# hideki1217/rusTfhe

Hardware: AMD Instinct MI355X
Metric: HomNAND gates/sec (whole node), N=1024 (higher is better)
Workload: dtype f64

## Files before the change

rustfhe_amd/csrc/rtfhe_body_pair.hpp:

```cpp
    constexpr int LOGN = 10;
    typedef Geo<LOGN> G;
    constexpr int N = G::N, P = G::P, R = G::R, NT = 128 * GATES;
    constexpr uint32_t M = decomp_mask(L, BGBIT);
    static_assert(L == 3, "three rows per side are held in registers");
    extern __shared__ __align__(16) unsigned char smem[];
    const int tid = threadIdx.x, lane = tid & 63;
    const int wave = __builtin_amdgcn_readfirstlane(tid >> 6);
    const int slot = wave % GATES;
    const int side = wave / GATES;
    cplx* tw = reinterpret_cast<cplx*>(smem);
    for (int idx = tid; idx < G::TW_TOTAL; idx += NT) tw[idx] = a.tw[idx];
    const cplx* twf = tw;
    const cplx* twi = tw + G::TW_DIR;

    const int g_raw = blockIdx.x * GATES + slot;
    const int g = g_raw < a.count ? g_raw : a.count - 1;
    const GateIo io = gate_io(a, g);
    const auto tv = tv_row(tvs, g, N);
    const bool live = g_raw < a.count && io.ok && tv.ok();

    unsigned char* gbase = smem + PairLds::TW + (size_t)slot * PairLds::gate_bytes(a.npad);
    uint32_t* accbuf = reinterpret_cast<uint32_t*>(gbase);
    uint32_t* abar = accbuf + 2 * N;
    double* xb0 = reinterpret_cast<double*>(gbase + (size_t)2 * N * 4 + (size_t)a.npad * 4);
    uint32_t* flags = reinterpret_cast<uint32_t*>(gbase + PairLds::gate_bytes(a.npad) - PairLds::FLAGS);
    if (lane == 0) flags[side] = 0u;
    const unsigned my_flag = (unsigned)__builtin_amdgcn_readfirstlane((int)(unsigned)(size_t)(__attribute__((address_space(3))) uint32_t*)(flags + side));
    const unsigned partner_flag = (unsigned)__builtin_amdgcn_readfirstlane((int)(unsigned)(size_t)(__attribute__((address_space(3))) uint32_t*)(flags + (1 - side)));
    double* xb1 = xb0 + 2 * G::XSLOTS;
    double* myx = side ? xb1 : xb0;
    cplx* hand0 = reinterpret_cast<cplx*>(xb0) + lane;
    cplx* hand1 = reinterpret_cast<cplx*>(xb1) + lane;
    uint32_t* poly = accbuf + side * N;

    const int n = a.n;
    {
        constexpr int SH = 32 - LOGN - 1;
        for (int i = lane + 64 * side; i <= n; i += 128) {
            const uint32_t t = gate_linear(io.op, io.p0[i], io.p1[i], i == n);
            if constexpr (decltype(tvs)::MANY) abar[i] = mod_switch<SH>(t, i == n, tv_shift(tvs));
            else abar[i] = (i == n) ? (t >> SH) : ((t + (1u << (SH - 1))) >> SH);
        }
    }
    __syncthreads();
    {
        const int bbar = (int)abar[n];
#pragma unroll
        for (int mm = 0; mm < 2 * R; mm++) {
            const int c = lane + 64 * mm;
            const int e = (c + bbar) & (2 * N - 1);
            if constexpr (decltype(tvs)::ENC) poly[c] = side ? tv_word_a<LOGN>(tv, e) : tv_word<LOGN>(tv, e);
            else poly[c] = side ? 0u : tv_word<LOGN>(tv, e);
        }
    }
    wave_lds_sync();
    uint32_t own[2 * R];
#pragma unroll
    for (int mm = 0; mm < 2 * R; mm++) own[mm] = poly[lane + 64 * mm];

#ifdef RTFHE_WG_STAMPS
    unsigned long long tsum[16] = {0, 0, 0, 0, 0, 0, 0, 0, 0, 0, 0, 0, 0, 0, 0, 0}, tprev = __builtin_amdgcn_s_memtime();
#define PAIR_STAMP(k) do { __builtin_amdgcn_sched_barrier(0); unsigned long long t_ = __builtin_amdgcn_s_memtime(); \
        asm volatile("s_waitcnt lgkmcnt(0)" ::: "memory"); tsum[k] += t_ - tprev; tprev = t_; __builtin_amdgcn_sched_barrier(0); } while (0)
#else
#define PAIR_STAMP(k) do { } while (0)
#endif
    const size_t trgsw_cplx = (size_t)2 * L * 2 * R * 64;
    cplx bA[R], bB[R];
    typedef unsigned int v4u __attribute__((ext_vector_type(4)));
    const __amdgpu_buffer_rsrc_t bk_rsrc = __builtin_amdgcn_make_buffer_rsrc(const_cast<cplx*>(a.bk), 0, 0x7fffffff, 0x00020000);
    const int lane16 = lane * 16;
    auto fetch = [&](cplx (&dst)[R], int step, int rc) {
        const size_t row = (size_t)step * trgsw_cplx + (size_t)((side * L + rc % L) * 2 + rc / L) * R * 64;
        const int s_lo = __builtin_amdgcn_readfirstlane((int)(row * sizeof(cplx)));
        const int s_hi = s_lo + (R / 2) * 64 * (int)sizeof(cplx);
        __builtin_amdgcn_sched_barrier(0);
#pragma unroll
        for (int m = 0; m < R / 2; m++) {
            const v4u v = __builtin_amdgcn_raw_buffer_load_b128(bk_rsrc, lane16 + m * 1024, s_lo, 0);
            dst[m] = make_double2(__longlong_as_double(((unsigned long long)v.y << 32) | v.x), __longlong_as_double(((unsigned long long)v.w << 32) | v.z));
        }
#pragma unroll
        for (int m = 0; m < R / 2; m++) {
            const v4u v = __builtin_amdgcn_raw_buffer_load_b128(bk_rsrc, lane16 + m * 1024, s_hi, 0);
            dst[R / 2 + m] = make_double2(__longlong_as_double(((unsigned long long)v.y << 32) | v.x), __longlong_as_double(((unsigned long long)v.w << 32) | v.z));
        }
        __builtin_amdgcn_sched_barrier(0);
    };
    if (a.steps > 0) {
        fetch(bA, 0, side ? 0 : 1);
        fetch(bB, 0, side ? 1 : 0);
    }
    constexpr int LOWER_AT = 2, RAISE_AT = 10;
    auto prio_point = [&](int point) {
        if (point == LOWER_AT) asm volatile("s_cmp_lg_u32 %0, 0\n\ts_cbranch_scc1 1f\n\ts_setprio 0\n1:" ::"s"(side) : "scc");
        if (point == RAISE_AT) asm volatile("s_cmp_lg_u32 %0, 0\n\ts_cbranch_scc1 1f\n\ts_setprio 2\n1:" ::"s"(side) : "scc");
    };
    if (side) __builtin_amdgcn_s_setprio(1); else __builtin_amdgcn_s_setprio(2);
#pragma unroll 1
    for (int i = 0; i < a.steps; i++) {
        const int r = __builtin_amdgcn_readfirstlane((int)abar[i]);
        const int nxt = (i + 1 < a.steps) ? i + 1 : i;
        int ln = lane;
        asm volatile("" : "+v"(ln));
        uint32_t u[2 * R];
#pragma unroll
        for (int mm = 0; mm < 2 * R; mm++) {
            const int c = ln + 64 * mm;
            u[mm] = ((rotated_coef<LOGN>(poly, c, r) - own[mm]) + M) ^ M;
        }
        PAIR_STAMP(0);
        double xr[L][R], xi[L][R];
#pragma unroll
        for (int jj = 0; jj < L; jj++) {
#pragma unroll
            for (int m = 0; m < R; m++) {
                xr[jj][m] = (double)decomp_digit(u[m], BGBIT, jj);
                xi[jj][m] = (double)decomp_digit(u[R + m], BGBIT, jj);
            }
        }
        auto pp1 = [&]() { prio_point(1); };
        fft_forward_multi_a<LOGN, L, true, decltype(pp1), true>(xr, xi, twf, myx, myx + G::XSLOTS, ln, pp1);
        prio_point(2);
        PAIR_STAMP(1);
        fft_forward_multi_b<LOGN, L, BOOT_TRIV>(xr, xi, twf);
        prio_point(5);
        PAIR_STAMP(3);

        double sre[R], sim[R];
        auto zero = [&]() {
#pragma unroll
            for (int m = 0; m < R; m++) { sre[m] = 0.0; sim[m] = 0.0; }
        };
        auto put = [&](cplx* h) {
#pragma unroll
            for (int m = 0; m < R; m++) h[m * 64] = make_double2(sre[m], sim[m]);
        };
        auto get = [&](const cplx* h) {
#pragma unroll
            for (int m = 0; m < R; m++) { const cplx v = h[m * 64]; sre[m] = v.x; sim[m] = v.y; }
        };

        if (side == 0) {
            mac_row_first<R>(sre, sim, bB, xr[0], xi[0]); fetch(bB, i, 2);
            mac_row<R>(sre, sim, bA, xr[1], xi[1]); fetch(bA, i, 3);
            mac_row<R>(sre, sim, bB, xr[2], xi[2]); fetch(bB, i, 4);
            put(hand0);
        }
        prio_point(6);
        PAIR_STAMP(4);
        flag_arrive(my_flag, 2u * (unsigned)i + 1u); flag_wait(partner_flag, 2u * (unsigned)i + 1u);
        prio_point(7);
        PAIR_STAMP(5);
        if (side == 0) zero(); else get(hand0);
        mac_row<R>(sre, sim, bA, xr[0], xi[0]); fetch(bA, i, side ? 2 : 5);
        mac_row<R>(sre, sim, bB, xr[1], xi[1]); fetch(bB, side ? i : nxt, side ? 3 : 0);
        mac_row<R>(sre, sim, bA, xr[2], xi[2]); fetch(bA, side ? i : nxt, side ? 4 : 1);
        put(side ? hand0 : hand1);
        prio_point(8);
        PAIR_STAMP(6);
        flag_arrive(my_flag, 2u * (unsigned)i + 2u); flag_wait(partner_flag, 2u * (unsigned)i + 2u);
        prio_point(9);
        PAIR_STAMP(7);
        if (side == 1) {
            get(hand1);
            mac_row<R>(sre, sim, bB, xr[0], xi[0]); fetch(bB, i, 5);
            mac_row<R>(sre, sim, bA, xr[1], xi[1]); fetch(bA, nxt, 0);
            mac_row<R>(sre, sim, bB, xr[2], xi[2]); fetch(bB, nxt, 1);
        } else {
            get(hand0);
        }
        PAIR_STAMP(8);

        fft_inverse<LOGN, 1, BOOT_TRIV>(sre, sim, twi, twi, myx, lane);
#pragma unroll
        for (int m = 0; m < R; m++) {
            const int c = lane + 64 * m;
            own[m] += trunc_to_torus(sre[m]);
            own[R + m] += trunc_to_torus(sim[m]);
            poly[c] = own[m];
            poly[c + P] = own[R + m];
        }
        wave_lds_sync();
        prio_point(10);
        PAIR_STAMP(9);
    }
    __builtin_amdgcn_s_setprio(0);
#ifdef RTFHE_WG_STAMPS
    if (a.dbg && blockIdx.x == 0 && lane == 0)
        for (int k = 0; k < 16; k++) a.dbg[wave * 16 + k] = tsum[k];
#endif

    if (a.mode == MODE_BLIND_ROTATE) {
        if (live) {
            uint32_t* o = a.out + (size_t)g * 2 * N + side * N;
            for (int c = lane; c < N; c += 64) o[c] = poly[c];
        }
        return;
    }

    if (side == 1) {
        uint32_t av[2 * R];
#pragma unroll
        for (int mm = 0; mm < 2 * R; mm++) av[mm] = poly[lane + 64 * mm];
        wave_lds_sync();
#pragma unroll
        for (int mm = 0; mm < 2 * R; mm++) {
            const int c = lane + 64 * mm;
            poly[(N - c) & (N - 1)] = (c == 0) ? av[mm] : (0u - av[mm]);
        }
    }
    __syncthreads();
    if (a.mode == MODE_EXTRACT) {
        if constexpr (decltype(tvs)::MANY) {
            if (live) many_extract<N>(a.ext, a.ext_first + g, tv_shift(tvs), accbuf, side * (N / 2) + lane, (side + 1) * (N / 2), 64, side ? -1 : lane);
            return;
        }
        if (live) {
            const int ge = a.ext_first + g;
            for (int c = side * (N / 2) + lane; c < (side + 1) * (N / 2); c += 64) *ext_slot(a.ext, ge, c, N) = accbuf[N + c];
            if (side == 0 && lane == 0) *ext_slot(a.ext, ge, N, N) = accbuf[0];
            for (int c = side * 64 + lane; c <= n; c += 128) io.out[c] = 0u;
        }
        return;
    }
    uint4 sum[KSQ];
    ks_accumulate<LOGN, KS_T, KS_BB, KSQ>(accbuf + N, side * (N / 2), (side + 1) * (N / 2), a.ksk, a.ksw, sum, lane);
    uint4* part = reinterpret_cast<uint4*>(xb1) + lane;
    if (side == 1) {
#pragma unroll
        for (int q = 0; q < KSQ; q++) part[q * 64] = sum[q];
    }
    __syncthreads();
    if (side == 0 && live) {
        const uint32_t bprime = accbuf[0];
        uint32_t* out = io.out;
#pragma unroll
        for (int q = 0; q < KSQ; q++) {
            const uint4 o = part[q * 64];
            const int col = 4 * (lane + 64 * q);
            const uint32_t s[4] = {sum[q].x + o.x, sum[q].y + o.y, sum[q].z + o.z, sum[q].w + o.w};
#pragma unroll
            for (int e = 0; e < 4; e++)
                if (col + e <= n) out[col + e] = ((col + e == n) ? bprime : 0u) - s[e];
        }
    }
```

rustfhe_amd/csrc/rtfhe_device.hpp:

```cpp
#pragma once

#include <hip/hip_runtime.h>
#include <stdint.h>

namespace rtfhe {

typedef double2 cplx;

constexpr bool BOOT_TRIV = true;

__host__ __device__ constexpr int ilog2(int v) { return v <= 1 ? 0 : 1 + ilog2(v >> 1); }

template <int LOGN>
struct Geo {
    static constexpr int N = 1 << LOGN;
    static constexpr int P = N / 2;
    static constexpr int LOGP = LOGN - 1;
    static constexpr int R = P / 64;
    static constexpr int LR = ilog2(R);
    static constexpr int LOW = LOGP - 2 * LR;
    static constexpr int NLOW = 1 << LOW;
    static_assert(LOW >= 2 && LOW <= LR, "supported: N = 1024, 2048");
    static constexpr int TW_TWIST = 0;
    static constexpr int TW_P1 = TW_TWIST + R * 64;
    static constexpr int TW_P2 = TW_P1 + (R - 1) * 64;
    static constexpr int TW_P3 = TW_P2 + (R - 1) * NLOW;
    static constexpr int TW_DIR = TW_P3 + (NLOW - 4);
    static constexpr int TW_TOTAL = 2 * TW_DIR;
    static constexpr int XSLOTS = P + 64;
    __host__ __device__ static constexpr int f1(int pos) { return pos + NLOW * (pos >> 6); }
    __host__ __device__ static constexpr int f2(int pos) { return pos + (pos >> LR); }
    __host__ __device__ static constexpr int pos1(int lane, int m) { return lane + 64 * m; }
    __host__ __device__ static constexpr int pos2(int lane, int m) {
        return ((lane >> LOW) << 6) | (m << LOW) | (lane & (NLOW - 1));
    }
    __host__ __device__ static constexpr int pos3(int lane, int m) { return (lane << LR) | m; }
};

__device__ __forceinline__ void wave_lds_sync() {
    __builtin_amdgcn_fence(__ATOMIC_RELEASE, "wavefront");
    __builtin_amdgcn_wave_barrier();
    __builtin_amdgcn_fence(__ATOMIC_ACQUIRE, "wavefront");
}

__device__ __forceinline__ void lds_st(double* p, double v) {
    __hip_atomic_store(p, v, __ATOMIC_RELAXED, __HIP_MEMORY_SCOPE_WAVEFRONT);
}
__device__ __forceinline__ double lds_ld(const double* p) {
    return __hip_atomic_load(p, __ATOMIC_RELAXED, __HIP_MEMORY_SCOPE_WAVEFRONT);
}
__device__ __forceinline__ void lds_st128(cplx* p, double re, double im) { *p = make_double2(re, im); }
__device__ __forceinline__ cplx lds_ld128(const cplx* p) { return *p; }


template <int CNT>
struct Tw {
    cplx w[CNT > 0 ? CNT : 1];
    __device__ __forceinline__ void load(const cplx* __restrict__ tw, int stride) {
#pragma unroll
        for (int e = 0; e < CNT; e++) w[e] = tw[e * stride];
    }
};

template <int R, int MB, bool TRIV0 = false>
__device__ __forceinline__ void fwd_stage_tw(double (&re)[R], double (&im)[R], const cplx* w) {
    constexpr int h = 1 << MB;
#pragma unroll
    for (int m = 0; m < R; m++) {
        if (m & h) continue;
        const int m1 = m | h, q = m & (h - 1);
        const double sr = re[m] + re[m1], si = im[m] + im[m1];
        const double dr = re[m] - re[m1], di = im[m] - im[m1];
        re[m] = sr; im[m] = si;
        if (TRIV0 && q == 0) { re[m1] = dr; im[m1] = di; continue; }
        double a = dr * w[q].x, b = di * w[q].y;
        re[m1] = a - b;
        a = dr * w[q].y; b = di * w[q].x;
        im[m1] = a + b;
    }
}

template <int R, int MB, bool CONJ = false, bool TRIV0 = false>
__device__ __forceinline__ void inv_stage_tw(double (&re)[R], double (&im)[R], const cplx* w) {
    constexpr int h = 1 << MB;
#pragma unroll
    for (int m = 0; m < R; m++) {
        if (m & h) continue;
        const int m1 = m | h, q = m & (h - 1);
        if (TRIV0 && q == 0) {
            const double ar = re[m], ai = im[m], tr = re[m1], ti = im[m1];
            re[m] = ar + tr; im[m] = ai + ti;
            re[m1] = ar - tr; im[m1] = ai - ti;
            continue;
        }
        const double t0 = re[m1] * w[q].x, t1 = re[m1] * w[q].y, t2 = im[m1] * w[q].x, t3 = im[m1] * w[q].y;
        const double tr = CONJ ? t0 + t3 : t0 - t3, ti = CONJ ? t2 - t1 : t1 + t2;
        const double ar = re[m], ai = im[m];
        re[m] = ar + tr; im[m] = ai + ti;
        re[m1] = ar - tr; im[m1] = ai - ti;
    }
}

template <int R>
__device__ __forceinline__ void stage_size2(double (&re)[R], double (&im)[R]) {
#pragma unroll
    for (int m = 0; m < R; m += 2) {
        const double r0 = re[m], r1 = re[m + 1], j0 = im[m], j1 = im[m + 1];
        re[m] = r0 + r1; re[m + 1] = r0 + (-r1);
        im[m] = j0 + j1; im[m + 1] = j0 + (-j1);
    }
}

template <int R>
__device__ __forceinline__ void fwd_stage_size4(double (&re)[R], double (&im)[R]) {
#pragma unroll
    for (int m = 0; m < R; m += 4) {
        const double r0 = re[m], r1 = re[m + 1], r2 = re[m + 2], r3 = re[m + 3];
        const double j0 = im[m], j1 = im[m + 1], j2 = im[m + 2], j3 = im[m + 3];
        re[m] = r0 + r2; re[m + 1] = r1 + r3; re[m + 2] = r0 + (-r2); re[m + 3] = (-j1) + j3;
        im[m] = j0 + j2; im[m + 1] = j1 + j3; im[m + 2] = j0 + (-j2); im[m + 3] = r1 + (-r3);
    }
}

template <int R>
__device__ __forceinline__ void inv_stage_size4(double (&re)[R], double (&im)[R]) {
#pragma unroll
    for (int m = 0; m < R; m += 4) {
        const double r0 = re[m], r1 = re[m + 1], r2 = re[m + 2], r3 = re[m + 3];
        const double j0 = im[m], j1 = im[m + 1], j2 = im[m + 2], j3 = im[m + 3];
        re[m] = r0 + r2; re[m + 1] = r1 + j3;    re[m + 2] = r0 + (-r2); re[m + 3] = r1 + (-j3);
        im[m] = j0 + j2; im[m + 1] = j1 + (-r3); im[m + 2] = j0 + (-j2); im[m + 3] = j1 + r3;
    }
}

template <int R>
__device__ __forceinline__ void twist_mul(double (&re)[R], double (&im)[R], const cplx* w) {
#pragma unroll
    for (int m = 0; m < R; m++) {
        const double rc = re[m] * w[m].x, ic = im[m] * w[m].x, rs = re[m] * w[m].y, is = im[m] * w[m].y;
        re[m] = rc - is;
        im[m] = ic + rs;
    }
}

// ... 112 lines not shown
        wave_lds_sync();
    }
}

template <int LOGN, int DUAL = 0>
__device__ __forceinline__ void fft_forward_a(double (&re)[Geo<LOGN>::R], double (&im)[Geo<LOGN>::R],
                                              const cplx* __restrict__ tw, double* __restrict__ xbuf, int lane,
                                              double* __restrict__ xim = nullptr) {
    typedef Geo<LOGN> G;
    constexpr int R = G::R;
    Tw<R> wt; Tw<R - 1> w1, w2;
    wt.load(tw + G::TW_TWIST + lane, 64);
    w1.load(tw + G::TW_P1 + lane, 64);
    twist_mul<R>(re, im, wt.w);
    P12<R, G::LR - 1>::fwd(re, im, w1.w);
    w2.load(tw + G::TW_P2 + (lane & (G::NLOW - 1)), G::NLOW);
    exchange<LOGN, 1, 2, DUAL>(re, im, xbuf, lane, xim);
    P12<R, G::LR - 1>::fwd(re, im, w2.w);
}
template <int LOGN, int DUAL = 0, bool TRIV = false>
__device__ __forceinline__ void fft_forward_b(double (&re)[Geo<LOGN>::R], double (&im)[Geo<LOGN>::R],
                                              const cplx* __restrict__ tw, double* __restrict__ xbuf, int lane,
                                              double* __restrict__ xim = nullptr) {
    typedef Geo<LOGN> G;
    Tw<G::NLOW - 4> w3;
    w3.load(tw + G::TW_P3, 1);
    exchange<LOGN, 2, 3, DUAL>(re, im, xbuf, lane, xim);
    P3<G::R, G::NLOW, G::LOW - 1, TRIV>::fwd(re, im, w3.w);
}
template <int LOGN, int DUAL = 0, bool TRIV = false>
__device__ __forceinline__ void fft_forward(double (&re)[Geo<LOGN>::R], double (&im)[Geo<LOGN>::R],
                                            const cplx* __restrict__ tw, double* __restrict__ xbuf, int lane,
                                            double* __restrict__ xim = nullptr) {
    fft_forward_a<LOGN, DUAL>(re, im, tw, xbuf, lane, xim);
    fft_forward_b<LOGN, DUAL, TRIV>(re, im, tw, xbuf, lane, xim);
}

template <int LOGN, int FROM, int TO, bool B128 = false>
struct XAffine {
    typedef Geo<LOGN> G;
    static_assert(G::LR == G::LOW, "N = 1024 geometry");
    static constexpr int R = G::R;
    static constexpr bool X12 = (FROM + TO == 3);
    __device__ __forceinline__ static int base(int layout, int lane) {
        return layout == 1 ? lane : layout == 2 ? (G::NLOW + 64) * (lane >> G::LOW) + (lane & (G::NLOW - 1)) : (R + 1) * lane;
    }
    __host__ __device__ static constexpr int stride(int layout) { return layout == 1 ? 64 + G::NLOW : layout == 2 ? (X12 ? G::NLOW : G::NLOW + 1) : 1; }
    __device__ __forceinline__ static void write(const double (&re)[R], const double (&im)[R], double* __restrict__ xbuf, double* __restrict__ xim, int lane) {
        const int bw = base(FROM, lane);
        constexpr int sw = stride(FROM);
        if constexpr (B128) {
            cplx* xc = reinterpret_cast<cplx*>(xbuf);
#pragma unroll
            for (int m = 0; m < R; m++) lds_st128(&xc[bw + sw * m], re[m], im[m]);
            return;
        }
#pragma unroll
        for (int m = 0; m < R; m++) lds_st(&xbuf[bw + sw * m], re[m]);
#pragma unroll
        for (int m = 0; m < R; m++) lds_st(&xim[bw + sw * m], im[m]);
    }
    template <int HALF>
    __device__ __forceinline__ static void read_half(double (&re)[R], double (&im)[R], const double* __restrict__ xbuf, const double* __restrict__ xim, int lane) {
        const int br = base(TO, lane);
        constexpr int sr = stride(TO);
        if constexpr (B128) {
            const cplx* xc = reinterpret_cast<const cplx*>(xbuf);
#pragma unroll
            for (int m = HALF * (R / 4); m < (HALF + 1) * (R / 4); m++) {
                const cplx a = lds_ld128(&xc[br + sr * m]), b = lds_ld128(&xc[br + sr * (m + R / 2)]);
                re[m] = a.x; im[m] = a.y; re[m + R / 2] = b.x; im[m + R / 2] = b.y;
            }
            return;
        }
#pragma unroll
        for (int m = HALF * (R / 4); m < (HALF + 1) * (R / 4); m++) {
            re[m] = lds_ld(&xbuf[br + sr * m]); re[m + R / 2] = lds_ld(&xbuf[br + sr * (m + R / 2)]);
            im[m] = lds_ld(&xim[br + sr * m]);  im[m + R / 2] = lds_ld(&xim[br + sr * (m + R / 2)]);
        }
    }
};

struct NoHook { __device__ __forceinline__ void operator()() const {} };
template <int LOGN, int NR, bool TWIST = true, typename HOOK = NoHook, bool INTERLEAVE = false, bool B128 = false>
__device__ __forceinline__ void fft_forward_multi_a(double (&re)[NR][Geo<LOGN>::R], double (&im)[NR][Geo<LOGN>::R],
                                                    const cplx* __restrict__ tw, double* __restrict__ xbuf, double* __restrict__ xim, int lane,
                                                    HOOK after_pass1 = HOOK()) {
    typedef Geo<LOGN> G;
    constexpr int R = G::R;
#pragma unroll
    for (int half = 0; half < (TWIST ? 2 : 0); half++) {
        cplx wt[R / 2];
#pragma unroll
        for (int m = 0; m < R / 2; m++) wt[m] = tw[G::TW_TWIST + lane + 64 * (half * (R / 2) + m)];
#pragma unroll
        for (int j = 0; j < NR; j++)
#pragma unroll
            for (int m = 0; m < R / 2; m++) {
                const int k = half * (R / 2) + m;
                const double rc = re[j][k] * wt[m].x, ic = im[j][k] * wt[m].x, rs = re[j][k] * wt[m].y, is = im[j][k] * wt[m].y;
                re[j][k] = rc - is;
                im[j][k] = ic + rs;
            }
    }
  if constexpr (INTERLEAVE) {
    static_assert(G::LR == 3, "three stages per pass");
    typedef XAffine<LOGN, 1, 2, B128> X1;
    typedef XAffine<LOGN, 2, 3, B128> X2;
    auto pass = [&](int j, const cplx* w, auto&& between0, auto&& between1) {
        fwd_stage_tw<R, 2>(re[j], im[j], w + (R - 8));
        __builtin_amdgcn_sched_barrier(0); between0(); __builtin_amdgcn_sched_barrier(0);
        fwd_stage_tw<R, 1>(re[j], im[j], w + (R - 4));
        __builtin_amdgcn_sched_barrier(0); between1(); __builtin_amdgcn_sched_barrier(0);
        fwd_stage_tw<R, 0>(re[j], im[j], w + (R - 2));
        __builtin_amdgcn_sched_barrier(0);
    };
    auto nothing = [] {};
    Tw<R - 1> w1;
    w1.load(tw + G::TW_P1 + lane, 64);
#pragma unroll
    for (int j = 0; j < NR; j++) {
        if (j == 0) pass(0, w1.w, nothing, nothing);
        else pass(j, w1.w, [&] { X1::template read_half<0>(re[j - 1], im[j - 1], xbuf, xim, lane); }, [&] { X1::template read_half<1>(re[j - 1], im[j - 1], xbuf, xim, lane); wave_lds_sync(); });
        X1::write(re[j], im[j], xbuf, xim, lane);
        wave_lds_sync();
    }
    after_pass1();
    Tw<R - 1> w2;
    w2.load(tw + G::TW_P2 + (lane & (G::NLOW - 1)), G::NLOW);
#pragma unroll
    for (int j = 0; j < NR; j++) {
        if (j == 0) pass(0, w2.w, [&] { X1::template read_half<0>(re[NR - 1], im[NR - 1], xbuf, xim, lane); }, [&] { X1::template read_half<1>(re[NR - 1], im[NR - 1], xbuf, xim, lane); wave_lds_sync(); });
        else pass(j, w2.w, [&] { X2::template read_half<0>(re[j - 1], im[j - 1], xbuf, xim, lane); }, [&] { X2::template read_half<1>(re[j - 1], im[j - 1], xbuf, xim, lane); wave_lds_sync(); });
        X2::write(re[j], im[j], xbuf, xim, lane);
        wave_lds_sync();
    }
    X2::template read_half<0>(re[NR - 1], im[NR - 1], xbuf, xim, lane);
    X2::template read_half<1>(re[NR - 1], im[NR - 1], xbuf, xim, lane);
    wave_lds_sync();
  } else {
    {
        Tw<R - 1> w1;
        w1.load(tw + G::TW_P1 + lane, 64);
#pragma unroll
        for (int j = 0; j < NR; j++) {
            P12<R, G::LR - 1>::fwd(re[j], im[j], w1.w);
            exchange<LOGN, 1, 2, B128 ? 2 : 1>(re[j], im[j], xbuf, lane, xim);
        }
    }
    after_pass1();
    Tw<R - 1> w2;
    w2.load(tw + G::TW_P2 + (lane & (G::NLOW - 1)), G::NLOW);
#pragma unroll
    for (int j = 0; j < NR; j++) {
        P12<R, G::LR - 1>::fwd(re[j], im[j], w2.w);
        exchange<LOGN, 2, 3, B128 ? 2 : 1>(re[j], im[j], xbuf, lane, xim);
    }
  }
}
template <int LOGN, int NR, bool TRIV = false>
__device__ __forceinline__ void fft_forward_multi_b(double (&re)[NR][Geo<LOGN>::R], double (&im)[NR][Geo<LOGN>::R],
                                                    const cplx* __restrict__ tw) {
    typedef Geo<LOGN> G;
    Tw<G::NLOW - 4> w3;
    w3.load(tw + G::TW_P3, 1);
#pragma unroll
    for (int j = 0; j < NR; j++) P3<G::R, G::NLOW, G::LOW - 1, TRIV>::fwd(re[j], im[j], w3.w);
}

template <int LOGN, int DUAL = 0, bool TRIV = false>
__device__ __forceinline__ void fft_inverse(double (&re)[Geo<LOGN>::R], double (&im)[Geo<LOGN>::R],
                                            const cplx* __restrict__ tw_small, const cplx* __restrict__ tw_big,
                                            double* __restrict__ xbuf, int lane, double* __restrict__ xim = nullptr) {
    typedef Geo<LOGN> G;
    constexpr int R = G::R;
    Tw<G::NLOW - 4> w3; Tw<R - 1> w2, w1; Tw<R> wt;
    w3.load(tw_small + G::TW_P3, 1);
    P3<R, G::NLOW, G::LOW - 1, TRIV>::template inv<false>(re, im, w3.w);
    w2.load(tw_small + G::TW_P2 + (lane & (G::NLOW - 1)), G::NLOW);
    exchange<LOGN, 3, 2, DUAL>(re, im, xbuf, lane, xim);
    P12<R, G::LR - 1>::inv(re, im, w2.w);
    w1.load(tw_big + G::TW_P1 + lane, 64);
    exchange<LOGN, 2, 1, DUAL>(re, im, xbuf, lane, xim);
    wt.load(tw_big + G::TW_TWIST + lane, 64);
    P12<R, G::LR - 1>::inv(re, im, w1.w);
    twist_mul<R>(re, im, wt.w);
}

template <int LOGN>
struct TwStage {
    typedef Geo<LOGN> G;
    static constexpr bool SPLIT = (LOGN >= 11);
    static constexpr int LDS_CPLX = SPLIT ? G::TW_DIR + (G::TW_DIR - G::TW_P2) : G::TW_TOTAL;
    __device__ __forceinline__ static void stage(cplx* __restrict__ lds, const cplx* __restrict__ global, int tid, int nthreads) {
        if constexpr (SPLIT) {
            for (int idx = tid; idx < G::TW_DIR; idx += nthreads) lds[idx] = global[idx];
            for (int idx = tid + G::TW_P2; idx < G::TW_DIR; idx += nthreads) lds[G::TW_DIR + idx - G::TW_P2] = global[G::TW_DIR + idx];
        } else {
            for (int idx = tid; idx < G::TW_TOTAL; idx += nthreads) lds[idx] = global[idx];
        }
    }
    __device__ __forceinline__ static const cplx* fwd(const cplx* lds) { return lds; }
    __device__ __forceinline__ static const cplx* inv_small(const cplx* lds) { return SPLIT ? lds + G::TW_DIR - G::TW_P2 : lds + G::TW_DIR; }
    __device__ __forceinline__ static const cplx* inv_big(const cplx* lds, const cplx* global) { return SPLIT ? global + G::TW_DIR : lds + G::TW_DIR; }
};

__device__ __forceinline__ uint32_t trunc_to_torus(double x) {
    const double t = __builtin_trunc(x);
    const double y = t + 6755399441055744.0;
    return (uint32_t)__double_as_longlong(y);
}

__device__ __forceinline__ uint32_t trunc_to_torus_wide(double x) {
    const double t = __builtin_trunc(x);
    if (!(__builtin_fabs(t) < 9223372036854775808.0)) return 0u;
    const double hi = __builtin_floor(t * 2.3283064365386963e-10);
    const double lo = __builtin_fma(hi, -4294967296.0, t);
    return (uint32_t)lo;
}

__host__ __device__ constexpr uint32_t decomp_mask(int l, int bits) {
    uint32_t u = 0;
    if (32 - l * bits != 0) {
        u += 1u << (32 - l * bits - 1);
        for (int i = l; i >= 1; i--) u += 1u << (32 - i * bits - 1);
    } else {
        for (int i = l - 1; i >= 1; i--) u += 1u << (32 - i * bits - 1);
    }
    return u;
}

__device__ __forceinline__ int32_t decomp_digit(uint32_t u, int bits, int j) {
    return __builtin_amdgcn_sbfe((int32_t)u, (uint32_t)(32 - bits * (j + 1)), (uint32_t)bits);
}


__device__ __forceinline__ void flag_arrive(unsigned flag, unsigned k) {
    unsigned t0, t1;
    asm volatile("v_mov_b32 %0, %2\n\tv_mov_b32 %1, %3\n\tds_write_b32 %0, %1" : "=&v"(t0), "=&v"(t1) : "s"(flag), "s"(k) : "memory");
}
__device__ __forceinline__ void flag_wait(unsigned flag, unsigned k) {
    unsigned v, t;
    asm volatile(
        "v_mov_b32 %0, %2\n"
        "1:\n\t"
        "ds_read_b32 %0, %0\n\t"
        "s_waitcnt lgkmcnt(0)\n\t"
        "v_readfirstlane_b32 %1, %0\n\t"
        "s_sub_i32 %1, %1, %3\n\t"
        "s_cmp_lt_i32 %1, 0\n\t"
        "s_cbranch_scc0 2f\n\t"
        "s_sleep 1\n\t"
        "v_mov_b32 %0, %2\n\t"
        "s_branch 1b\n"
        "2:"
        : "=&v"(v), "=&s"(t)
        : "s"(flag), "s"(k)
        : "memory", "scc");
}
template <int LOGN>
__device__ __forceinline__ uint32_t rotated_coef(const uint32_t* __restrict__ p, int c, int r) {
    constexpr int N = 1 << LOGN;
    const int e = (c - r) & (2 * N - 1);
    const uint32_t v = p[e & (N - 1)];
    return (e >> LOGN) ? (0u - v) : v;
}

}
```

rustfhe_amd/csrc/rtfhe_kernels_pair.hpp:

```cpp
#pragma once

#include "rtfhe_kernels.hpp"


namespace rtfhe {

__device__ __forceinline__ void lds_barrier() {
    asm volatile("s_waitcnt lgkmcnt(0)\n\ts_barrier" ::: "memory");
}

__device__ __forceinline__ void pair_sync(unsigned my_flag_addr, unsigned partner_flag_addr, unsigned k) {
    asm volatile("ds_write_b32 %0, %1" ::"v"(my_flag_addr), "v"(k) : "memory");
    unsigned v;
    do {
        asm volatile("ds_read_b32 %0, %1\n\ts_waitcnt lgkmcnt(0)" : "=v"(v) : "v"(partner_flag_addr) : "memory");
        v = (unsigned)__builtin_amdgcn_readfirstlane((int)v);
    } while ((int)(v - k) < 0);
}

__device__ __forceinline__ void pair_arrive(unsigned my_flag_addr, unsigned k) {
    asm volatile("ds_write_b32 %0, %1" ::"v"(my_flag_addr), "v"(k) : "memory");
}
__device__ __forceinline__ void pair_wait(unsigned partner_flag_addr, unsigned k) {
    unsigned v;
    do {
        asm volatile("ds_read_b32 %0, %1\n\ts_waitcnt lgkmcnt(0)" : "=v"(v) : "v"(partner_flag_addr) : "memory");
        v = (unsigned)__builtin_amdgcn_readfirstlane((int)v);
    } while ((int)(v - k) < 0);
}

__device__ __forceinline__ void pair_wait_opaque(unsigned partner_flag_addr, unsigned k) {
    unsigned v, t;
    asm volatile(
        "1:\n\t"
        "ds_read_b32 %0, %2\n\t"
        "s_waitcnt lgkmcnt(0)\n\t"
        "v_readfirstlane_b32 %1, %0\n\t"
        "s_sub_i32 %1, %1, %3\n\t"
        "s_cmp_lt_i32 %1, 0\n\t"
        "s_cbranch_scc1 1b"
        : "=&v"(v), "=&s"(t)
        : "v"(partner_flag_addr), "s"(k)
        : "memory", "scc");
}

__device__ __forceinline__ void pair_wait_opaque_prio3(unsigned partner_flag_addr, unsigned k) {
    unsigned v, t;
    asm volatile(
        "1:\n\t"
        "ds_read_b32 %0, %2\n\t"
        "s_waitcnt lgkmcnt(0)\n\t"
        "v_readfirstlane_b32 %1, %0\n\t"
        "s_sub_i32 %1, %1, %3\n\t"
        "s_cmp_lt_i32 %1, 0\n\t"
        "s_cbranch_scc1 1b\n\t"
        "s_setprio 3"
        : "=&v"(v), "=&s"(t)
        : "v"(partner_flag_addr), "s"(k)
        : "memory", "scc");
}

template <int R>
__device__ __forceinline__ void mac_row_first(double (&sre)[R], double (&sim)[R], const cplx (&b)[R], const double (&re)[R], const double (&im)[R]) {
#pragma unroll
    for (int m = 0; m < R; m++) {
        const double ii = b[m].y * im[m], rr = b[m].x * re[m], ri = b[m].x * im[m], ir = b[m].y * re[m];
        sre[m] = rr - ii;
        sim[m] = ir + ri;
    }
}

template <int R>
__device__ __forceinline__ void mac_row(double (&sre)[R], double (&sim)[R], const cplx (&b)[R], const double (&re)[R], const double (&im)[R]) {
#pragma unroll
    for (int m = 0; m < R; m++) {
        const double ii = b[m].y * im[m], rr = b[m].x * re[m], ri = b[m].x * im[m], ir = b[m].y * re[m];
        sre[m] = sre[m] + (rr - ii);
        sim[m] = sim[m] + (ir + ri);
    }
}

struct PairLds {
    typedef Geo<10> G;
    static constexpr size_t TW = (size_t)G::TW_TOTAL * sizeof(cplx);
    static constexpr size_t XB = (size_t)2 * G::XSLOTS * sizeof(double);
    static_assert(XB >= (size_t)G::P * sizeof(cplx), "an exchange buffer pair must hold one spectrum");
    static constexpr size_t FLAGS = 16;
    __host__ __device__ static constexpr size_t gate_bytes(int npad) { return (size_t)2 * G::N * 4 + (size_t)npad * 4 + 2 * XB + FLAGS; }
    __host__ __device__ static constexpr size_t bytes(int gates, int npad) { return TW + (size_t)gates * gate_bytes(npad); }
};

template <int L, int BGBIT, int KS_T, int KS_BB, int KSQ, int GATES>
__global__ __launch_bounds__(128 * GATES, 1) void k_bootstrap_pair(const BootstrapArgs a) {
    const TvGate tvs{};
#include "rtfhe_body_pair.hpp"
}
template <int L, int BGBIT, int KS_T, int KS_BB, int KSQ, int GATES>
__global__ __launch_bounds__(128 * GATES, 1) void k_pbs_pair(const LutArgs<BootstrapArgs> p) {
    const BootstrapArgs& a = p.base;
    const TvLut tvs = tv_lut(p, a.fault);
#include "rtfhe_body_pair.hpp"
}
template <int L, int BGBIT, int KS_T, int KS_BB, int KSQ, int GATES>
__global__ __launch_bounds__(128 * GATES, 1) void k_pbs_many_pair(const ManyArgs<BootstrapArgs> p) {
    const BootstrapArgs& a = p.base;
    const TvMany tvs = tv_many(p, a.fault);
#include "rtfhe_body_pair.hpp"
}
template <int L, int BGBIT, int KS_T, int KS_BB, int KSQ, int GATES>
__global__ __launch_bounds__(128 * GATES, 1) void k_pbs_enc_pair(const ManyArgs<BootstrapArgs> p) {
    const BootstrapArgs& a = p.base;
    const TvEnc tvs = tv_enc(p, a.fault);
#include "rtfhe_body_pair.hpp"
}

}
```

rustfhe_amd/csrc/rtfhe_kernels_pair_rr.hpp:

```cpp
#pragma once

#include "rtfhe_kernels_pair.hpp"

namespace rtfhe {

struct PairRrLds {
    typedef Geo<10> G;
    static constexpr int SLOTS = 4, GMAX = 6;
    static constexpr size_t TW = PairLds::TW, XB = PairLds::XB;
    static constexpr size_t SLOT = 2 * XB + 16;
    static constexpr size_t DONE = 64;
    __host__ __device__ static constexpr size_t gate_bytes(int npad) { return (size_t)2 * G::N * 4 + ((size_t)npad * 2 + 15) / 16 * 16; }
    __host__ __device__ static constexpr size_t bytes(int gates, int npad) { return TW + SLOTS * SLOT + DONE + (size_t)gates * gate_bytes(npad); }
};

template <int L, int BGBIT, int KS_T, int KS_BB, int KSQ>
__global__ __launch_bounds__(512, 1) void k_bootstrap_pair_rr(const BootstrapArgs a) {
    const TvGate tvs{};
#include "rtfhe_body_pair_rr.hpp"
}
template <int L, int BGBIT, int KS_T, int KS_BB, int KSQ>
__global__ __launch_bounds__(512, 1) void k_pbs_pair_rr(const LutArgs<BootstrapArgs> p) {
    const BootstrapArgs& a = p.base;
    const TvLut tvs = tv_lut(p, a.fault);
#include "rtfhe_body_pair_rr.hpp"
}
template <int L, int BGBIT, int KS_T, int KS_BB, int KSQ>
__global__ __launch_bounds__(512, 1) void k_pbs_many_pair_rr(const ManyArgs<BootstrapArgs> p) {
    const BootstrapArgs& a = p.base;
    const TvMany tvs = tv_many(p, a.fault);
#include "rtfhe_body_pair_rr.hpp"
}
template <int L, int BGBIT, int KS_T, int KS_BB, int KSQ>
__global__ __launch_bounds__(512, 1) void k_pbs_enc_pair_rr(const ManyArgs<BootstrapArgs> p) {
    const BootstrapArgs& a = p.base;
    const TvEnc tvs = tv_enc(p, a.fault);
#include "rtfhe_body_pair_rr.hpp"
}

}
```

Baseline: 155,800.

## Keep only small FFT twiddle tables in LDS, stream large ones from global

The pair bootstrap kernel now copies only the pass-2/pass-3 twiddle tables (forward and inverse) into LDS. The large twist and pass-1 tables are read per lane directly from global memory through buffer loads. This shrinks the LDS footprint per workgroup, which may allow more gates per block or better occupancy. The cost is extra global/L2 traffic and latency on every FFT, and the rr kernel keeps the full table size.

```diff
diff --git a/rustfhe_amd/csrc/rtfhe_body_pair.hpp b/rustfhe_amd/csrc/rtfhe_body_pair.hpp
--- a/rustfhe_amd/csrc/rtfhe_body_pair.hpp
+++ b/rustfhe_amd/csrc/rtfhe_body_pair.hpp
@@ -9,9 +9,10 @@
     const int slot = wave % GATES;
     const int side = wave / GATES;
     cplx* tw = reinterpret_cast<cplx*>(smem);
-    for (int idx = tid; idx < G::TW_TOTAL; idx += NT) tw[idx] = a.tw[idx];
-    const cplx* twf = tw;
-    const cplx* twi = tw + G::TW_DIR;
+    for (int idx = tid; idx < 2 * PairLds::TW_SMALL; idx += NT)
+        tw[idx] = a.tw[idx < PairLds::TW_SMALL ? G::TW_P2 + idx : G::TW_DIR + G::TW_P2 + idx - PairLds::TW_SMALL];
+    const cplx* twf_small = tw;
+    const cplx* twi_small = tw + PairLds::TW_SMALL;
 
     const int g_raw = blockIdx.x * GATES + slot;
     const int g = g_raw < a.count ? g_raw : a.count - 1;
@@ -70,6 +71,8 @@
     typedef unsigned int v4u __attribute__((ext_vector_type(4)));
     const __amdgpu_buffer_rsrc_t bk_rsrc = __builtin_amdgcn_make_buffer_rsrc(const_cast<cplx*>(a.bk), 0, 0x7fffffff, 0x00020000);
     const int lane16 = lane * 16;
+    const __amdgpu_buffer_rsrc_t tw_rsrc = __builtin_amdgcn_make_buffer_rsrc(const_cast<cplx*>(a.tw), 0, G::TW_TOTAL * (int)sizeof(cplx), 0x00020000);
+    const TwBuf twf_big{tw_rsrc, lane16, 0}, twi_big{tw_rsrc, lane16, G::TW_DIR * (int)sizeof(cplx)};
     auto fetch = [&](cplx (&dst)[R], int step, int rc) {
         const size_t row = (size_t)step * trgsw_cplx + (size_t)((side * L + rc % L) * 2 + rc / L) * R * 64;
         const int s_lo = __builtin_amdgcn_readfirstlane((int)(row * sizeof(cplx)));
@@ -120,10 +123,10 @@
             }
         }
         auto pp1 = [&]() { prio_point(1); };
-        fft_forward_multi_a<LOGN, L, true, decltype(pp1), true>(xr, xi, twf, myx, myx + G::XSLOTS, ln, pp1);
+        fft_forward_multi_a_from<LOGN, L, true, decltype(pp1), true, false>(xr, xi, twf_big, TwLds{twf_small + (ln & (G::NLOW - 1))}, myx, myx + G::XSLOTS, ln, pp1);
         prio_point(2);
         PAIR_STAMP(1);
-        fft_forward_multi_b<LOGN, L, BOOT_TRIV>(xr, xi, twf);
+        fft_forward_multi_b_from<LOGN, L, BOOT_TRIV>(xr, xi, twf_small + (G::TW_P3 - G::TW_P2));
         prio_point(5);
         PAIR_STAMP(3);
 
@@ -172,7 +175,7 @@
         }
         PAIR_STAMP(8);
 
-        fft_inverse<LOGN, 1, BOOT_TRIV>(sre, sim, twi, twi, myx, lane);
+        fft_inverse_from<LOGN, 1, BOOT_TRIV>(sre, sim, twi_small + (G::TW_P3 - G::TW_P2), TwLds{twi_small + (lane & (G::NLOW - 1))}, twi_big, myx, lane);
 #pragma unroll
         for (int m = 0; m < R; m++) {
             const int c = lane + 64 * m;
diff --git a/rustfhe_amd/csrc/rtfhe_device.hpp b/rustfhe_amd/csrc/rtfhe_device.hpp
--- a/rustfhe_amd/csrc/rtfhe_device.hpp
+++ b/rustfhe_amd/csrc/rtfhe_device.hpp
@@ -60,6 +60,27 @@
 #pragma unroll
         for (int e = 0; e < CNT; e++) w[e] = tw[e * stride];
     }
+    template <typename SRC>
+    __device__ __forceinline__ void load_from(const SRC& src, int off, int stride) {
+#pragma unroll
+        for (int e = 0; e < CNT; e++) w[e] = src(off + e * stride);
+    }
+};
+
+struct TwLds {
+    const cplx* p;
+    __device__ __forceinline__ cplx operator()(int off) const { return p[off]; }
+};
+struct TwBuf {
+    typedef unsigned int v4u __attribute__((ext_vector_type(4)));
+    __amdgpu_buffer_rsrc_t rsrc;
+    int voff;
+    int base;
+    __device__ __forceinline__ cplx operator()(int off) const {
+        const int byte = base + off * (int)sizeof(cplx);
+        const v4u v = __builtin_amdgcn_raw_buffer_load_b128(rsrc, voff + (byte & 4095), byte & ~4095, 0);
+        return make_double2(__longlong_as_double(((unsigned long long)v.y << 32) | v.x), __longlong_as_double(((unsigned long long)v.w << 32) | v.z));
+    }
 };
 
 template <int R, int MB, bool TRIV0 = false>
@@ -338,17 +359,17 @@
 };
 
 struct NoHook { __device__ __forceinline__ void operator()() const {} };
-template <int LOGN, int NR, bool TWIST = true, typename HOOK = NoHook, bool INTERLEAVE = false, bool B128 = false>
-__device__ __forceinline__ void fft_forward_multi_a(double (&re)[NR][Geo<LOGN>::R], double (&im)[NR][Geo<LOGN>::R],
-                                                    const cplx* __restrict__ tw, double* __restrict__ xbuf, double* __restrict__ xim, int lane,
-                                                    HOOK after_pass1 = HOOK()) {
+template <int LOGN, int NR, bool TWIST, typename HOOK, bool INTERLEAVE, bool B128, typename BIG, typename P2>
+__device__ __forceinline__ void fft_forward_multi_a_from(double (&re)[NR][Geo<LOGN>::R], double (&im)[NR][Geo<LOGN>::R],
+                                                         const BIG& big, const P2& p2, double* __restrict__ xbuf, double* __restrict__ xim, int lane,
+                                                         HOOK after_pass1) {
     typedef Geo<LOGN> G;
     constexpr int R = G::R;
 #pragma unroll
     for (int half = 0; half < (TWIST ? 2 : 0); half++) {
         cplx wt[R / 2];
 #pragma unroll
-        for (int m = 0; m < R / 2; m++) wt[m] = tw[G::TW_TWIST + lane + 64 * (half * (R / 2) + m)];
+        for (int m = 0; m < R / 2; m++) wt[m] = big(G::TW_TWIST + 64 * (half * (R / 2) + m));
 #pragma unroll
         for (int j = 0; j < NR; j++)
 #pragma unroll
@@ -373,7 +394,7 @@
     };
     auto nothing = [] {};
     Tw<R - 1> w1;
-    w1.load(tw + G::TW_P1 + lane, 64);
+    w1.load_from(big, G::TW_P1, 64);
 #pragma unroll
     for (int j = 0; j < NR; j++) {
         if (j == 0) pass(0, w1.w, nothing, nothing);
@@ -383,7 +404,7 @@
     }
     after_pass1();
     Tw<R - 1> w2;
-    w2.load(tw + G::TW_P2 + (lane & (G::NLOW - 1)), G::NLOW);
+    w2.load_from(p2, 0, G::NLOW);
 #pragma unroll
     for (int j = 0; j < NR; j++) {
         if (j == 0) pass(0, w2.w, [&] { X1::template read_half<0>(re[NR - 1], im[NR - 1], xbuf, xim, lane); }, [&] { X1::template read_half<1>(re[NR - 1], im[NR - 1], xbuf, xim, lane); wave_lds_sync(); });
@@ -397,7 +418,7 @@
   } else {
     {
         Tw<R - 1> w1;
-        w1.load(tw + G::TW_P1 + lane, 64);
+        w1.load_from(big, G::TW_P1, 64);
 #pragma unroll
         for (int j = 0; j < NR; j++) {
             P12<R, G::LR - 1>::fwd(re[j], im[j], w1.w);
@@ -406,7 +427,7 @@
     }
     after_pass1();
     Tw<R - 1> w2;
-    w2.load(tw + G::TW_P2 + (lane & (G::NLOW - 1)), G::NLOW);
+    w2.load_from(p2, 0, G::NLOW);
 #pragma unroll
     for (int j = 0; j < NR; j++) {
         P12<R, G::LR - 1>::fwd(re[j], im[j], w2.w);
@@ -414,33 +435,52 @@
     }
   }
 }
+template <int LOGN, int NR, bool TWIST = true, typename HOOK = NoHook, bool INTERLEAVE = false, bool B128 = false>
+__device__ __forceinline__ void fft_forward_multi_a(double (&re)[NR][Geo<LOGN>::R], double (&im)[NR][Geo<LOGN>::R],
+                                                    const cplx* __restrict__ tw, double* __restrict__ xbuf, double* __restrict__ xim, int lane,
+                                                    HOOK after_pass1 = HOOK()) {
+    typedef Geo<LOGN> G;
+    fft_forward_multi_a_from<LOGN, NR, TWIST, HOOK, INTERLEAVE, B128>(re, im, TwLds{tw + lane}, TwLds{tw + G::TW_P2 + (lane & (G::NLOW - 1))}, xbuf, xim, lane, after_pass1);
+}
+template <int LOGN, int NR, bool TRIV = false>
+__device__ __forceinline__ void fft_forward_multi_b_from(double (&re)[NR][Geo<LOGN>::R], double (&im)[NR][Geo<LOGN>::R],
+                                                         const cplx* __restrict__ tw_p3) {
+    typedef Geo<LOGN> G;
+    Tw<G::NLOW - 4> w3;
+    w3.load(tw_p3, 1);
+#pragma unroll
+    for (int j = 0; j < NR; j++) P3<G::R, G::NLOW, G::LOW - 1, TRIV>::fwd(re[j], im[j], w3.w);
+}
 template <int LOGN, int NR, bool TRIV = false>
 __device__ __forceinline__ void fft_forward_multi_b(double (&re)[NR][Geo<LOGN>::R], double (&im)[NR][Geo<LOGN>::R],
                                                     const cplx* __restrict__ tw) {
-    typedef Geo<LOGN> G;
-    Tw<G::NLOW - 4> w3;
-    w3.load(tw + G::TW_P3, 1);
-#pragma unroll
-    for (int j = 0; j < NR; j++) P3<G::R, G::NLOW, G::LOW - 1, TRIV>::fwd(re[j], im[j], w3.w);
-}
-
+    fft_forward_multi_b_from<LOGN, NR, TRIV>(re, im, tw + Geo<LOGN>::TW_P3);
+}
+
+template <int LOGN, int DUAL, bool TRIV, typename BIG, typename P2>
+__device__ __forceinline__ void fft_inverse_from(double (&re)[Geo<LOGN>::R], double (&im)[Geo<LOGN>::R],
+                                                 const cplx* __restrict__ tw_p3, const P2& p2, const BIG& big,
+                                                 double* __restrict__ xbuf, int lane, double* __restrict__ xim = nullptr) {
+    typedef Geo<LOGN> G;
+    constexpr int R = G::R;
+    Tw<G::NLOW - 4> w3; Tw<R - 1> w2, w1; Tw<R> wt;
+    w3.load(tw_p3, 1);
+    P3<R, G::NLOW, G::LOW - 1, TRIV>::template inv<false>(re, im, w3.w);
+    w2.load_from(p2, 0, G::NLOW);
+    exchange<LOGN, 3, 2, DUAL>(re, im, xbuf, lane, xim);
+    P12<R, G::LR - 1>::inv(re, im, w2.w);
+    w1.load_from(big, G::TW_P1, 64);
+    exchange<LOGN, 2, 1, DUAL>(re, im, xbuf, lane, xim);
+    wt.load_from(big, G::TW_TWIST, 64);
+    P12<R, G::LR - 1>::inv(re, im, w1.w);
+    twist_mul<R>(re, im, wt.w);
+}
 template <int LOGN, int DUAL = 0, bool TRIV = false>
 __device__ __forceinline__ void fft_inverse(double (&re)[Geo<LOGN>::R], double (&im)[Geo<LOGN>::R],
                                             const cplx* __restrict__ tw_small, const cplx* __restrict__ tw_big,
                                             double* __restrict__ xbuf, int lane, double* __restrict__ xim = nullptr) {
     typedef Geo<LOGN> G;
-    constexpr int R = G::R;
-    Tw<G::NLOW - 4> w3; Tw<R - 1> w2, w1; Tw<R> wt;
-    w3.load(tw_small + G::TW_P3, 1);
-    P3<R, G::NLOW, G::LOW - 1, TRIV>::template inv<false>(re, im, w3.w);
-    w2.load(tw_small + G::TW_P2 + (lane & (G::NLOW - 1)), G::NLOW);
-    exchange<LOGN, 3, 2, DUAL>(re, im, xbuf, lane, xim);
-    P12<R, G::LR - 1>::inv(re, im, w2.w);
-    w1.load(tw_big + G::TW_P1 + lane, 64);
-    exchange<LOGN, 2, 1, DUAL>(re, im, xbuf, lane, xim);
-    wt.load(tw_big + G::TW_TWIST + lane, 64);
-    P12<R, G::LR - 1>::inv(re, im, w1.w);
-    twist_mul<R>(re, im, wt.w);
+    fft_inverse_from<LOGN, DUAL, TRIV>(re, im, tw_small + G::TW_P3, TwLds{tw_small + G::TW_P2 + (lane & (G::NLOW - 1))}, TwLds{tw_big + lane}, xbuf, lane, xim);
 }
 
 template <int LOGN>
diff --git a/rustfhe_amd/csrc/rtfhe_kernels_pair.hpp b/rustfhe_amd/csrc/rtfhe_kernels_pair.hpp
--- a/rustfhe_amd/csrc/rtfhe_kernels_pair.hpp
+++ b/rustfhe_amd/csrc/rtfhe_kernels_pair.hpp
@@ -82,7 +82,9 @@
 
 struct PairLds {
     typedef Geo<10> G;
-    static constexpr size_t TW = (size_t)G::TW_TOTAL * sizeof(cplx);
+    static constexpr int TW_SMALL = G::TW_DIR - G::TW_P2;
+    static constexpr size_t TW = (size_t)2 * TW_SMALL * sizeof(cplx);
+    static constexpr size_t TW_FULL = (size_t)G::TW_TOTAL * sizeof(cplx);
     static constexpr size_t XB = (size_t)2 * G::XSLOTS * sizeof(double);
     static_assert(XB >= (size_t)G::P * sizeof(cplx), "an exchange buffer pair must hold one spectrum");
     static constexpr size_t FLAGS = 16;
diff --git a/rustfhe_amd/csrc/rtfhe_kernels_pair_rr.hpp b/rustfhe_amd/csrc/rtfhe_kernels_pair_rr.hpp
--- a/rustfhe_amd/csrc/rtfhe_kernels_pair_rr.hpp
+++ b/rustfhe_amd/csrc/rtfhe_kernels_pair_rr.hpp
@@ -7,7 +7,7 @@
 struct PairRrLds {
     typedef Geo<10> G;
     static constexpr int SLOTS = 4, GMAX = 6;
-    static constexpr size_t TW = PairLds::TW, XB = PairLds::XB;
+    static constexpr size_t TW = PairLds::TW_FULL, XB = PairLds::XB;
     static constexpr size_t SLOT = 2 * XB + 16;
     static constexpr size_t DONE = 64;
     __host__ __device__ static constexpr size_t gate_bytes(int npad) { return (size_t)2 * G::N * 4 + ((size_t)npad * 2 + 15) / 16 * 16; }
```

After: 153,200. -1.7%, worse.

## Prefetch rotation amounts in blocks and issue next-step poly gather early

Applied to the files above, without the earlier changes.

Rotation amounts abar[i] are now read from LDS four at a time with a ds_read_b128, issued during the inverse-FFT phase and held in scalar registers. The next step's rotated-coefficient gather from poly is issued at the end of each iteration, right after the LDS sync, instead of at the top of the next one. This moves LDS read latency off the critical path at the start of each blind-rotate step. In exchange it holds more registers live across the loop and relies on custom inline asm with a manual lgkmcnt wait, plus the abar buffer having four-element alignment and padding.

```diff
diff --git a/rustfhe_amd/csrc/rtfhe_body_pair.hpp b/rustfhe_amd/csrc/rtfhe_body_pair.hpp
--- a/rustfhe_amd/csrc/rtfhe_body_pair.hpp
+++ b/rustfhe_amd/csrc/rtfhe_body_pair.hpp
@@ -97,17 +97,43 @@
         if (point == RAISE_AT) asm volatile("s_cmp_lg_u32 %0, 0\n\ts_cbranch_scc1 1f\n\ts_setprio 2\n1:" ::"s"(side) : "scc");
     };
     if (side) __builtin_amdgcn_s_setprio(1); else __builtin_amdgcn_s_setprio(2);
+    const unsigned abar_lds = (unsigned)__builtin_amdgcn_readfirstlane((int)(unsigned)(size_t)(__attribute__((address_space(3))) uint32_t*)abar);
+    int r, rq0, rq1, rq2;
+    {
+        const uint4 b4 = *reinterpret_cast<const uint4*>(abar);
+        r = __builtin_amdgcn_readfirstlane((int)b4.x);
+        rq0 = __builtin_amdgcn_readfirstlane((int)b4.y);
+        rq1 = __builtin_amdgcn_readfirstlane((int)b4.z);
+        rq2 = __builtin_amdgcn_readfirstlane((int)b4.w);
+    }
+    uint32_t gv[2 * R];
+    int e0;
+    auto gather_addr = [&](const uint32_t* (&ga)[2 * R], int ln_, int r_) {
+        e0 = ln_ - r_;
+#pragma unroll
+        for (int mm = 0; mm < 2 * R; mm++) ga[mm] = poly + ((e0 + 64 * mm) & (N - 1));
+    };
+    auto gather = [&](const uint32_t* const (&ga)[2 * R]) {
+#pragma unroll
+        for (int mm = 0; mm < 2 * R; mm++) gv[mm] = *ga[mm];
+    };
+    {
+        int ln0 = lane;
+        const uint32_t* ga[2 * R];
+        asm volatile("" : "+v"(ln0));
+        gather_addr(ga, ln0, r);
+        gather(ga);
+    }
 #pragma unroll 1
     for (int i = 0; i < a.steps; i++) {
-        const int r = __builtin_amdgcn_readfirstlane((int)abar[i]);
         const int nxt = (i + 1 < a.steps) ? i + 1 : i;
         int ln = lane;
         asm volatile("" : "+v"(ln));
         uint32_t u[2 * R];
 #pragma unroll
         for (int mm = 0; mm < 2 * R; mm++) {
-            const int c = ln + 64 * mm;
-            u[mm] = ((rotated_coef<LOGN>(poly, c, r) - own[mm]) + M) ^ M;
+            const uint32_t v = (((e0 + 64 * mm) >> LOGN) & 1) ? (0u - gv[mm]) : gv[mm];
+            u[mm] = ((v - own[mm]) + M) ^ M;
         }
         PAIR_STAMP(0);
         double xr[L][R], xi[L][R];
@@ -162,6 +188,8 @@
         flag_arrive(my_flag, 2u * (unsigned)i + 2u); flag_wait(partner_flag, 2u * (unsigned)i + 2u);
         prio_point(9);
         PAIR_STAMP(7);
+        rot_block_t blk;
+        rot_block_issue(blk, abar_lds + 4u * (unsigned)(i + 1), i + 1);
         if (side == 1) {
             get(hand1);
             mac_row<R>(sre, sim, bB, xr[0], xi[0]); fetch(bB, i, 5);
@@ -171,19 +199,34 @@
             get(hand0);
         }
         PAIR_STAMP(8);
-
         fft_inverse<LOGN, 1, BOOT_TRIV>(sre, sim, twi, twi, myx, lane);
+        rot_block_land(blk);
+        const bool fresh = ((i + 1) & 3) == 0;
+        const int b0 = __builtin_amdgcn_readfirstlane((int)blk.x), b1 = __builtin_amdgcn_readfirstlane((int)blk.y);
+        const int b2 = __builtin_amdgcn_readfirstlane((int)blk.z), b3 = __builtin_amdgcn_readfirstlane((int)blk.w);
+        r = fresh ? b0 : rq0;
+        rq0 = fresh ? b1 : rq1;
+        rq1 = fresh ? b2 : rq2;
+        rq2 = fresh ? b3 : rq2;
+        const uint32_t* ga[2 * R];
+        gather_addr(ga, ln, r);
+#pragma unroll
+        for (int m = 0; m < R; m++) {
+            own[m] += trunc_to_torus(sre[m]);
+            own[R + m] += trunc_to_torus(sim[m]);
+        }
+        __builtin_amdgcn_sched_barrier(0);
 #pragma unroll
         for (int m = 0; m < R; m++) {
             const int c = lane + 64 * m;
-            own[m] += trunc_to_torus(sre[m]);
-            own[R + m] += trunc_to_torus(sim[m]);
             poly[c] = own[m];
             poly[c + P] = own[R + m];
         }
         wave_lds_sync();
         prio_point(10);
         PAIR_STAMP(9);
+        gather(ga);
+        asm volatile("" ::: "memory");
     }
     __builtin_amdgcn_s_setprio(0);
 #ifdef RTFHE_WG_STAMPS
diff --git a/rustfhe_amd/csrc/rtfhe_device.hpp b/rustfhe_amd/csrc/rtfhe_device.hpp
--- a/rustfhe_amd/csrc/rtfhe_device.hpp
+++ b/rustfhe_amd/csrc/rtfhe_device.hpp
@@ -514,6 +514,23 @@
         : "s"(flag), "s"(k)
         : "memory", "scc");
 }
+typedef unsigned int rot_block_t __attribute__((ext_vector_type(4)));
+__device__ __forceinline__ void rot_block_issue(rot_block_t& blk, unsigned addr, int j) {
+    unsigned va, t;
+    asm volatile(
+        "s_and_b32 %2, %3, 3\n\t"
+        "s_cmp_lg_u32 %2, 0\n\t"
+        "s_cbranch_scc1 1f\n\t"
+        "v_mov_b32 %1, %4\n\t"
+        "ds_read_b128 %0, %1\n"
+        "1:"
+        : "=&v"(blk), "=&v"(va), "=&s"(t)
+        : "s"(j), "s"(addr)
+        : "scc");
+}
+__device__ __forceinline__ void rot_block_land(rot_block_t& blk) {
+    asm volatile("s_waitcnt lgkmcnt(0)" : "+v"(blk));
+}
 template <int LOGN>
 __device__ __forceinline__ uint32_t rotated_coef(const uint32_t* __restrict__ p, int c, int r) {
     constexpr int N = 1 << LOGN;
```

Result: slower. 153,800 before, 149,900 after (-2.5%).

## Rotate accumulator in registers via ds_bpermute instead of LDS round-trip

Applied to the files above, without the earlier changes.

Replaces the per-step LDS store of the accumulator and the rotated LDS reads with a register-level negacyclic rotation. The high bits of the rotation pick one of 32 compile-time register permutations through a switch, and the low bits become a cross-lane ds_bpermute with a wrap select and sign handling. The accumulator is written back to LDS only once, after the blind-rotate loop. This removes a per-iteration LDS write plus wave sync and a gather read. In exchange it adds a 32-way switch with fully unrolled bodies, which increases code size and instruction-cache pressure and may raise register use.

```diff
diff --git a/rustfhe_amd/csrc/rtfhe_body_pair.hpp b/rustfhe_amd/csrc/rtfhe_body_pair.hpp
--- a/rustfhe_amd/csrc/rtfhe_body_pair.hpp
+++ b/rustfhe_amd/csrc/rtfhe_body_pair.hpp
@@ -104,10 +104,9 @@
         int ln = lane;
         asm volatile("" : "+v"(ln));
         uint32_t u[2 * R];
-#pragma unroll
-        for (int mm = 0; mm < 2 * R; mm++) {
-            const int c = ln + 64 * mm;
-            u[mm] = ((rotated_coef<LOGN>(poly, c, r) - own[mm]) + M) ^ M;
+        {
+            const int r_lo = r & 63, r_hi = (r >> 6) & 31;
+            pair_rotate_diff_any<M>(u, own, r_hi, ((ln - r_lo) & 63) << 2, ln >= 64 - r_lo);
         }
         PAIR_STAMP(0);
         double xr[L][R], xi[L][R];
@@ -175,17 +174,16 @@
         fft_inverse<LOGN, 1, BOOT_TRIV>(sre, sim, twi, twi, myx, lane);
 #pragma unroll
         for (int m = 0; m < R; m++) {
-            const int c = lane + 64 * m;
             own[m] += trunc_to_torus(sre[m]);
             own[R + m] += trunc_to_torus(sim[m]);
-            poly[c] = own[m];
-            poly[c + P] = own[R + m];
-        }
-        wave_lds_sync();
+        }
         prio_point(10);
         PAIR_STAMP(9);
     }
     __builtin_amdgcn_s_setprio(0);
+#pragma unroll
+    for (int mm = 0; mm < 2 * R; mm++) poly[lane + 64 * mm] = own[mm];
+    wave_lds_sync();
 #ifdef RTFHE_WG_STAMPS
     if (a.dbg && blockIdx.x == 0 && lane == 0)
         for (int k = 0; k < 16; k++) a.dbg[wave * 16 + k] = tsum[k];
diff --git a/rustfhe_amd/csrc/rtfhe_kernels_pair.hpp b/rustfhe_amd/csrc/rtfhe_kernels_pair.hpp
--- a/rustfhe_amd/csrc/rtfhe_kernels_pair.hpp
+++ b/rustfhe_amd/csrc/rtfhe_kernels_pair.hpp
@@ -1,4 +1,6 @@
 #pragma once
+
+#include <utility>
 
 #include "rtfhe_kernels.hpp"
 
@@ -80,6 +82,43 @@
     }
 }
 
+template <int RH, int MM, uint32_t M, int NR>
+__device__ __forceinline__ uint32_t pair_rotate_diff_one(const uint32_t (&own)[NR], int src4, bool srcb) {
+    constexpr int W = 2 * NR, K = (MM - RH + W) % W, KB = (K + W - 1) % W;
+    constexpr bool NEG = K >= NR, NEGB = KB >= NR;
+    const uint32_t x = own[K % NR], xb = own[KB % NR];
+    if constexpr (NEG == NEGB) {
+        const uint32_t v = (uint32_t)__builtin_amdgcn_ds_bpermute(src4, (int)(srcb ? xb : x));
+        return NEG ? ((M - (v + own[MM])) ^ M) : (((v - own[MM]) + M) ^ M);
+    } else {
+        const uint32_t sx = NEG ? 0u - x : x, sxb = NEGB ? 0u - xb : xb;
+        const uint32_t v = (uint32_t)__builtin_amdgcn_ds_bpermute(src4, (int)(srcb ? sxb : sx));
+        return ((v - own[MM]) + M) ^ M;
+    }
+}
+template <int RH, uint32_t M, int NR, int... MM>
+__device__ __forceinline__ void pair_rotate_diff_seq(uint32_t (&u)[NR], const uint32_t (&own)[NR], int src4, bool srcb, std::integer_sequence<int, MM...>) {
+    ((u[MM] = pair_rotate_diff_one<RH, MM, M>(own, src4, srcb)), ...);
+}
+template <int RH, uint32_t M, int NR>
+__device__ __forceinline__ void pair_rotate_diff(uint32_t (&u)[NR], const uint32_t (&own)[NR], int src4, bool srcb) {
+    static_assert(NR == 16, "1024 coefficients in 16 registers of 64 lanes");
+    pair_rotate_diff_seq<RH, M>(u, own, src4, srcb, std::make_integer_sequence<int, NR>{});
+}
+
+template <uint32_t M, int NR>
+__device__ __forceinline__ void pair_rotate_diff_any(uint32_t (&u)[NR], const uint32_t (&own)[NR], int r_hi, int src4, bool srcb) {
+#define RTFHE_ROT_CASE(k) case k: pair_rotate_diff<k, M>(u, own, src4, srcb); break;
+#define RTFHE_ROT_CASE4(k) RTFHE_ROT_CASE(k) RTFHE_ROT_CASE(k + 1) RTFHE_ROT_CASE(k + 2) RTFHE_ROT_CASE(k + 3)
+    switch (r_hi) {
+        RTFHE_ROT_CASE4(0) RTFHE_ROT_CASE4(4) RTFHE_ROT_CASE4(8) RTFHE_ROT_CASE4(12)
+        RTFHE_ROT_CASE4(16) RTFHE_ROT_CASE4(20) RTFHE_ROT_CASE4(24) RTFHE_ROT_CASE4(28)
+        default: __builtin_unreachable();
+    }
+#undef RTFHE_ROT_CASE4
+#undef RTFHE_ROT_CASE
+}
+
 struct PairLds {
     typedef Geo<10> G;
     static constexpr size_t TW = (size_t)G::TW_TOTAL * sizeof(cplx);
```

Result: no change. 157,600 before, 158,600 after, median of 6 (+0.6%).
